# struan-robertson/shoeprint-image-retrieval

Measured on AMD Instinct MI355X. Metric: query x gallery NCC pairs/sec, higher is better.
Workload: dtype f32; 1 GPU; config 2: WVU2019-shaped VGG16 conv3_3 NCC: Q=100 x G=1500 (1500/GPU), features [256,128,64] stored as float32, rotations/scales none, queries signal 1 / noise 126; method=fft, gallery_chunk=1500, storage=float32, parallelism=gallery-shard x1, streams=1

## Files before the change

shoeprint-image-retrieval_amd/csrc/ncc_pair6.hip:

```cpp
#include <cstdlib>

#include "fft_core.h"
#include "ncc_fft_cfg.h"

namespace spr {
namespace {

#ifndef SPR_ABL
#define SPR_ABL 0
#endif
#ifndef SPR_X6
#define SPR_X6 0
#endif
#ifdef SPR_STAMPS
constexpr int kStampPoints = 12, kStampChannels = 8, kStampFirst = 8;
__device__ unsigned long long g_stamps[12 * kStampChannels * kStampPoints];
#define SPR_STAMP(i) st[i] = __builtin_amdgcn_s_memtime()
#else
#define SPR_STAMP(i)
#endif

constexpr int kTileQ6 = 16, kTileG6 = 16;

struct Pair6Args {
  int channels, nq, ng;
  int ih, iw;
  int inv_per_chan;
  int accumulate;
  int tile0;
  int tiles_g;
  int prio_mode;
  unsigned q_flags_off, g_flags_off;
};

template <int DIR>
__device__ __forceinline__ void pfa12(cf (&x)[12]) {
  constexpr float h = DIR > 0 ? 0.86602540378443860f : -0.86602540378443860f;
  cf a[3][4];
#pragma unroll
  for (int n2 = 0; n2 < 4; ++n2) {
    const cf x0 = x[(3 * n2) % 12], x1 = x[(4 + 3 * n2) % 12], x2 = x[(8 + 3 * n2) % 12];
    const cf s = x1 + x2, d = x1 - x2;
    const cf m = x0 - 0.5f * s;
    a[0][n2] = x0 + s;
    a[1][n2] = pk_iaxpy_u(d, h, m);
    a[2][n2] = pk_iaxpy_u(d, -h, m);
  }
#pragma unroll
  for (int k1 = 0; k1 < 3; ++k1) {
    const cf e0 = a[k1][0] + a[k1][2], e1 = a[k1][0] - a[k1][2];
    const cf o0 = a[k1][1] + a[k1][3], o1 = a[k1][1] - a[k1][3];
    x[(4 * k1) % 12] = e0 + o0;
    x[(4 * k1 + 18) % 12] = e0 - o0;
    x[(4 * k1 + 9) % 12] = DIR > 0 ? pk_add_i(e1, o1) : pk_sub_i(e1, o1);
    x[(4 * k1 + 27) % 12] = DIR > 0 ? pk_sub_i(e1, o1) : pk_add_i(e1, o1);
  }
}

template <class C>
struct Six {
  static_assert(C::SIX == 1 && C::EH == 12 && C::TGH == 16 && C::NW == 96 && C::NT == 384, "192 x 96 on six waves");
  static constexpr int NT = C::NT, WAVES = NT / 64;
  static constexpr int RS = 139;
  static __device__ __forceinline__ int xpos(int u) {
    if (SPR_X6 == 0) return (u / 21) * RS + u % 21;
    const int a = u < 21 ? 0 : (u < 32 ? 1 : (u < 43 ? 2 : (u < 53 ? 1 : 2)));
    const int o = u < 21 ? u : (u < 32 ? u - 11 : (u < 43 ? u - 22 : (u < 53 ? u - 43 : (u == 53 ? 9 : u - 54))));
    return a * RS + o;
  }
  static constexpr int XR = 65;
  static constexpr int XROWS = 6;
  static constexpr int kXbWave = XROWS * XR + 6;
  static constexpr int kImgOff = 0;
  static constexpr int kImgBytes = C::COLS * RS * 8;
  static constexpr int kXbOff = kImgOff + kImgBytes;
  static constexpr int kNyqOff = kXbOff + WAVES * kXbWave * 8;
  static constexpr int kHalfBytes = kNyqOff + 2 * 2 * C::NH * 8;
  static constexpr int kRedOff = 2 * kHalfBytes;
  static constexpr int kPeakOff = kRedOff + 128;
  static constexpr int kTwOff = kPeakOff + 64;
  static constexpr int kCtabOff = kTwOff + C::NH * 8;
  static constexpr int kListOff = kCtabOff + 48 * 4;
  static constexpr int kLdsBytes = kListOff;
  static_assert(kLdsBytes + 2 * 2 * 1024 <= 160 * 1024, "one workgroup of two pairs per CU, up to 1024 channels");
  static_assert(kXbOff % 8 == 0 && kNyqOff % 8 == 0 && kHalfBytes % 16 == 0 && kTwOff % 8 == 0 && kCtabOff % 8 == 0, "");
};

template <class C, bool PEAKS>
__global__ void __launch_bounds__(2 * C::NT, 3)
pair6_kernel(Pair6Args g, const unsigned char* __restrict__ pq, size_t q_item_bytes,
             const unsigned char* __restrict__ pg, size_t g_item_bytes, float* __restrict__ scores, long long ld,
             long long col0, float* __restrict__ maps_out, const cf* __restrict__ tw_h,
             const float* __restrict__ ctab, int32_t* __restrict__ peak_yx, int32_t* __restrict__ peak_tag,
             int32_t tag) {
  using S = Six<C>;
  constexpr int NT = S::NT, RS = S::RS, XR = S::XR;
  constexpr int H2 = C::EH / 2;

  constexpr int kWgPerTile = kTileQ6 * kTileG6 / 2;
  const int tile = g.tile0 + static_cast<int>(blockIdx.x) / kWgPerTile;
  const int within = static_cast<int>(blockIdx.x) % kWgPerTile;
  const int tq = tile / g.tiles_g, tg = tile - tq * g.tiles_g;
  const int half = uniform(static_cast<int>(threadIdx.x) >= NT ? 1 : 0);
  const int q_first = tq * kTileQ6 + 2 * (within >> 4);
  const int gi_item = tg * kTileG6 + 2 * (within & 7) + ((within >> 3) & 1);
  if (q_first >= g.nq || gi_item >= g.ng) return;
  const bool live = q_first + half < g.nq;
  const int qi = live ? q_first + half : q_first;

  unsigned char* lds = dyn_lds();
  unsigned char* hl = lds + half * S::kHalfBytes;
  float* red = reinterpret_cast<float*>(lds + S::kRedOff) + half * 8;
  unsigned* bar = reinterpret_cast<unsigned*>(lds + S::kRedOff + 64) + half * 8;
  unsigned* nlive_p = bar + 2;
  unsigned bar_target = 0;
  cf* R = reinterpret_cast<cf*>(hl + S::kImgOff);
  cf* nyq = reinterpret_cast<cf*>(hl + S::kNyqOff);
  cf* twt_h = reinterpret_cast<cf*>(lds + S::kTwOff);
  cf* ctab2 = reinterpret_cast<cf*>(lds + S::kCtabOff);
  unsigned short* chan = reinterpret_cast<unsigned short*>(lds + S::kListOff) + half * g.channels;

  const int tid0 = static_cast<int>(threadIdx.x) - half * NT;
  const int wv = uniform(tid0 >> 6);
  cf* xb = reinterpret_cast<cf*>(hl + S::kXbOff) + wv * S::kXbWave;

  const unsigned char* g_item = pg + static_cast<size_t>(gi_item) * g_item_bytes;
  const unsigned char* q_item = pq + static_cast<size_t>(qi) * q_item_bytes;

  if (tid0 == 0) *bar = 0u;
  if (half == 0) {
    for (int k = tid0; k < C::NH; k += NT) twt_h[k] = cconj(tw_h[(k / C::TGH) * (k % C::TGH)]);
    if (tid0 < 24) {
      const int a = (tid0 / 3) * 2, t = tid0 % 3;
      ctab2[tid0] = cmake(ctab[(3 * a + 16 * t) % 48], ctab[(3 * (a + 1) + 16 * t) % 48]);
    }
  }
  for (int k = tid0; k < g.channels; k += NT)
    chan[k] = (q_item[g.q_flags_off + k] | g_item[g.g_flags_off + k]) ? 0xFFFFu : static_cast<unsigned short>(k);
  __syncthreads();
  if (tid0 == 0) {
    int n = 0;
    for (int k = 0; k < g.channels; ++k) {
      const unsigned short v = chan[k];
      if (v != 0xFFFFu) chan[n++] = v;
    }
    if (n == 0) chan[0] = 0;
    *nlive_p = static_cast<unsigned>(n);
  }
  __syncthreads();
  const int nlive = uniform(static_cast<int>(*nlive_p));
  const int last_i = nlive > 0 ? nlive - 1 : 0;
  auto chan_at = [&](int i) { return static_cast<int>(chan[i < last_i ? i : last_i]); };

  float4 nxt[2 * H2];
  cf nyq_g, nyq_q;
  const BufRsrc g_rs = make_rsrc(g_item, g_item_bytes), q_rs = make_rsrc(q_item, q_item_bytes);
  const unsigned voff16 = static_cast<unsigned>(tid0) * 16u;
  const unsigned voff_nyq = static_cast<unsigned>(tid0 % C::NH) * 8u + C::kNyqOffset * 8u;
  constexpr unsigned kChanBytes = C::kSpecPerChan * 8u;
  const unsigned inv_base = static_cast<unsigned>(g.channels) * kChanBytes;
  auto issue_unit = [&](int c, int rc) {
    const unsigned so = static_cast<unsigned>(c) * kChanBytes + static_cast<unsigned>(rc * H2 * NT * 16);
    if (SPR_ABL == 1) {
      for (int mm = 0; mm < 2 * H2; ++mm) nxt[mm] = make_float4(0.001f * so, 0.5f, 0.25f, 0.125f);
      return;
    }
#pragma unroll
    for (int mm = 0; mm < H2; ++mm) {
      nxt[mm] = buf_ld16(g_rs, voff16, so + mm * NT * 16);
      nxt[H2 + mm] = buf_ld16(q_rs, voff16, so + mm * NT * 16);
    }
  };
  auto issue_nyq = [&](int c) {
    const unsigned so = static_cast<unsigned>(c) * kChanBytes;
    nyq_g = buf_ld8(g_rs, voff_nyq, so);
    nyq_q = buf_ld8(q_rs, voff_nyq, so);
  };
  static_assert(2 * C::NH == NT, "one Nyquist value per lane");

#ifndef SPR_EMU
  {
    const int gw = half * S::WAVES + wv;
    if (g.prio_mode == 2 && (gw == 4 || gw == 5 || gw >= 8)) __builtin_amdgcn_s_setprio(1);
  }
#endif
  cf acc[6][2];
#pragma unroll
  for (int pp = 0; pp < 6; ++pp) acc[pp][0] = acc[pp][1] = cmake(0.0f, 0.0f);

  issue_nyq(chan_at(0));
  nyq[tid0] = tid0 < C::NH ? nyq_g : nyq_q;
  issue_nyq(chan_at(1));
  nyq[NT + tid0] = tid0 < C::NH ? nyq_g : nyq_q;
  issue_unit(chan_at(0), 0);
  __syncthreads();

  for (int ci = 0; ci < nlive; ++ci) {
    const int c = chan_at(ci), c1 = chan_at(ci + 1), c2 = chan_at(ci + 2);
#ifdef SPR_STAMPS
    unsigned long long st[kStampPoints] = {};
#endif
    SPR_STAMP(0);
    const int tid = opaque(tid0);
    const int lane = tid & 63;
    const int g4 = lane >> 4, tc = lane & 15;

    auto product = [&](cf (&z)[12], int rc) {
#pragma unroll
      for (int mm = 0; mm < H2; ++mm) {
        const float4 a = nxt[mm], b = nxt[H2 + mm];
        z[2 * mm] = cmul(cmake(a.x, a.y), cmake(b.x, b.y));
        z[2 * mm + 1] = cmul(cmake(a.z, a.w), cmake(b.z, b.w));
      }
      if (rc == 0 && tid < 16) {
        const cf* nq = nyq + (ci & 1) * NT;
#pragma unroll
        for (int m = 0; m < 12; ++m) {
          const int k1 = tc + 16 * m;
          z[m] = pk_add_i(z[m], cmul(nq[k1], nq[C::NH + k1]));
        }
      }
    };
    auto stage12 = [&](cf (&z)[12]) {
      pfa12<+1>(z);
#pragma unroll
      for (int p = 1; p < 12; ++p) z[p] = cmul(z[p], twt_h[p * 16 + tc]);
    };
    auto exchange = [&](const cf (&z)[12], cf (&y)[16], int rc) {
      const int own0 = (rc * 24 + 4 * wv) * RS;
      const int xb_el = (S::kXbOff - S::kImgOff) / 8 + wv * S::kXbWave;
      const int skew = ((xb_el + 6 - own0) % 32 + 32) % 32;
      cf* own = R + own0 + skew;
      wave_sync();
      cf* w0 = xb + lane;
      cf* w1 = own + lane;
      if (SPR_ABL != 3) {
#pragma unroll
        for (int p = 0; p < 6; ++p) w0[p * XR] = z[p];
#pragma unroll
        for (int p = 6; p < 12; ++p) w1[(p - 6) * XR] = z[p];
      }
      wave_sync();
      const cf* rd = (tc < 6 ? xb + tc * XR : (tc < 12 ? own + (tc - 6) * XR : xb)) + 16 * g4;
#pragma unroll
      for (int tt = 0; tt < 16; ++tt) y[tt] = rd[tt];
    };
    auto part2 = [&](cf (&y)[16], int rc) {
      wave_sync();
      if (tc < 12) {
        if (SPR_ABL != 4) Dft<16, +1>::run(y);
        cf* col = R + (rc * 24 + 4 * wv + g4) * RS + tc;
        if (SPR_ABL != 3) {
#pragma unroll
          for (int s = 0; s < 11; ++s) col[12 * s] = y[s];
        }
      }
    };

    {
      cf za[12], ya[16], zb[12], yb[16];
      issue_nyq(c2);
      product(za, 0);
      issue_unit(c, 1);
      stage12(za);
#pragma unroll
      for (int p = 0; p < 12; ++p) pin(za[p]);
      SPR_STAMP(1);
      bar_target += S::WAVES;
      if (SPR_ABL != 2) group_barrier(bar, bar_target);
      SPR_STAMP(2);
      product(zb, 1);
      sched_fence();
      exchange(za, ya, 0);
      sched_fence();
      stage12(zb);
      sched_fence();
      issue_unit(c1, 0);
      SPR_STAMP(3);
      part2(ya, 0);
      SPR_STAMP(4);
      exchange(zb, yb, 1);
      SPR_STAMP(5);
      part2(yb, 1);
      SPR_STAMP(6);
    }
    bar_target += S::WAVES;
    if (SPR_ABL != 2) group_barrier(bar, bar_target);
    SPR_STAMP(7);
    {
      const int grp = lane / 3;
      const int t3 = lane - 3 * grp;
      const int grp_r = grp < C::kRowGroups ? grp : C::kRowGroups - 1;
      const int row = wv * C::kRowGroups + grp_r;
      const int tm = t3 == 0 ? 0 : 3 - t3;
      const cf* dbase = R + t3 * RS + row;
      const cf* mbase = R + tm * RS + row;
      const cf* cc = ctab2 + t3;
      cf z[16];
#pragma unroll
      for (int a2 = 0; a2 < 8; ++a2) {
        const cf ck = cc[a2 * 3];
#pragma unroll
        for (int h = 0; h < 2; ++h) {
          const int a = 2 * a2 + h;
          const int ra = (3 * a) % 16, rm = (3 * ((16 - a) % 16)) % 16;
          const cf av = dbase[3 * ra * RS];
          const cf bv = mbase[3 * rm * RS];
          cf v = h == 0 ? pk_conj_iaxpy<0>(av, ck, bv) : pk_conj_iaxpy<1>(av, ck, bv);
          if (a == 0) {
            const cf v0 = cmake(av.x + av.y, av.x - av.y);
            v = t3 == 0 ? v0 : v;
          }
          z[a] = v;
        }
      }
      SPR_STAMP(8);
      if (SPR_ABL != 4) Dft<16, +1>::run(z);
      sched_fence();
      float4 iv[6];
      const unsigned so_inv = inv_base + static_cast<unsigned>(c) * static_cast<unsigned>(g.inv_per_chan) * 4u;
#pragma unroll
      for (int pp = 0; pp < 6; ++pp)
        iv[pp] = SPR_ABL == 1 ? make_float4(1.f, 1.f, 1.f, 1.f) : buf_ld16(g_rs, voff16, so_inv + pp * NT * 16);
      const float kH = 0.86602540378443860f;
      const cf kl = t3 == 1 ? cmake(-0.5f, kH) : cmake(1.0f, 0.0f);
      const cf hb = t3 == 0 ? cmake(kH, 0.0f) : cmake(-kH, 0.0f);
      cf* wx = R + S::xpos(lane < 63 ? lane : 62) + wv * C::kRowGroups;
      const cf* rxt[3];
#pragma unroll
      for (int tt = 0; tt < 3; ++tt) rxt[tt] = R + S::xpos(3 * grp_r + tt) + wv * C::kRowGroups;
      wave_sync();
      if (lane < 63 && SPR_ABL != 3) {
#pragma unroll
        for (int r = 0; r < 16; ++r) wx[3 * r * RS] = z[r];
      }
      SPR_STAMP(9);
      wave_sync();
      cf yv[6][3];
#pragma unroll
      for (int pp = 0; pp < 6; ++pp)
#pragma unroll
        for (int tt = 0; tt < 3; ++tt)
          yv[pp][tt] = pp < 5 ? rxt[tt][(9 * pp + 3 * t3) * RS] : rxt[tt][45 * RS];
#pragma unroll
      for (int pp = 0; pp < 6; ++pp) {
        const cf y0 = yv[pp][0], y1 = yv[pp][1], y2 = yv[pp][2];
        const cf s = y1 + y2, d = y1 - y2;
        const cf m = y0 - 0.5f * s;
        const cf ob = pk_iaxpy<0>(d, hb, m);
        const cf oa = pk_iaxpy<1>(d, kl, pk_axpy<0>(s, kl, y0));
        const cf ia = cmake(iv[pp].x, iv[pp].y), ib = cmake(iv[pp].z, iv[pp].w);
        acc[pp][0] = oa * ia + acc[pp][0];
        acc[pp][1] = ob * ib + acc[pp][1];
        if (maps_out && half == 0) {
          const int n1 = t3 + 3 * pp;
          const int real_row = wv * C::kRowGroups + grp;
          if (n1 < 16 && grp < C::kRowGroups && real_row < g.ih) {
            const int ma = t3 == 2 ? n1 + 16 : n1, mb = t3 == 2 ? n1 : n1 + 16;
            float* dst = maps_out + (static_cast<size_t>(c) * g.ih + real_row) * g.iw;
            if (2 * ma < g.iw) dst[2 * ma] = oa.x * ia.x;
            if (2 * ma + 1 < g.iw) dst[2 * ma + 1] = oa.y * ia.y;
            if (2 * mb < g.iw) dst[2 * mb] = ob.x * ib.x;
            if (2 * mb + 1 < g.iw) dst[2 * mb + 1] = ob.y * ib.y;
          }
        }
      }
      nyq[(ci & 1) * NT + tid] = tid < C::NH ? nyq_g : nyq_q;
    }
    SPR_STAMP(10);
#ifdef SPR_STAMPS
    if (blockIdx.x == 777 && (tid0 & 63) == 0 && ci >= kStampFirst && ci < kStampFirst + kStampChannels) {
      for (int i = 0; i < kStampPoints; ++i)
        g_stamps[((half * 6 + wv) * kStampChannels + (ci - kStampFirst)) * kStampPoints + i] = st[i];
    }
#endif
  }

  if constexpr (PEAKS) {
    const int lane = tid0 & 63;
    const int grp = lane / 3, t3 = lane - 3 * grp;
    const int real_row = wv * C::kRowGroups + grp;
    const bool row_ok = grp < C::kRowGroups && real_row < g.ih;
    float best = 0.0f;
    int where = kNoPeak;
#pragma unroll
    for (int pp = 0; pp < 6; ++pp) {
      const int n1 = t3 + 3 * pp;
      const int ma = t3 == 2 ? n1 + 16 : n1, mb = t3 == 2 ? n1 : n1 + 16;
      const int at = real_row << 16;
      if (row_ok && n1 < 16) {
        if (2 * ma < g.iw) peak_take(best, where, acc[pp][0].x, at | (2 * ma));
        if (2 * ma + 1 < g.iw) peak_take(best, where, acc[pp][0].y, at | (2 * ma + 1));
        if (2 * mb < g.iw) peak_take(best, where, acc[pp][1].x, at | (2 * mb));
        if (2 * mb + 1 < g.iw) peak_take(best, where, acc[pp][1].y, at | (2 * mb + 1));
      }
    }
    wave_peak(best, where);
    int* red_pos = reinterpret_cast<int*>(lds + S::kPeakOff) + half * 8;
    if ((tid0 & 63) == 0) {
      red[wv] = best;
      red_pos[wv] = where;
    }
    __syncthreads();
    if (tid0 == 0 && live) {
      float b = red[0];
      int p = red_pos[0];
      for (int w = 1; w < S::WAVES; ++w) peak_take(b, p, red[w], red_pos[w]);
      store_peak(scores, peak_yx, peak_tag, static_cast<size_t>(qi) * ld + col0 + gi_item, b / static_cast<float>(g.channels), p,
                 tag, g.accumulate);
    }
    return;
  }
  float best = 0.0f;
#pragma unroll
  for (int pp = 0; pp < 6; ++pp) {
    best = fmaxf(best, fmaxf(fmaxf(acc[pp][0].x, acc[pp][0].y), fmaxf(acc[pp][1].x, acc[pp][1].y)));
  }
  for (int m = 32; m >= 1; m >>= 1) best = fmaxf(best, shfl_xor(best, m));
  if ((tid0 & 63) == 0) red[wv] = best;
  __syncthreads();
  if (tid0 == 0 && scores && live) {
    float b = red[0];
    for (int w = 1; w < S::WAVES; ++w) b = fmaxf(b, red[w]);
    const float s = b / static_cast<float>(g.channels);
    float* dst = scores + static_cast<size_t>(qi) * ld + col0 + gi_item;
    const float prev = g.accumulate ? *dst : 0.0f;
    *dst = s > prev ? s : prev;
  }
}

using C6 = Cfg<12, 16, 12, 8, 384, 5, 2, 1>;

}

#ifdef SPR_STAMPS
extern "C" int spr_debug_read_stamps(unsigned long long* host, int n) {
  return hipMemcpyFromSymbol(host, HIP_SYMBOL(g_stamps), sizeof(unsigned long long) * n) == hipSuccess ? 0 : -1;
}
#endif

size_t pair6_lds_bytes() { return Six<C6>::kLdsBytes; }
int pair6_max_rows() { return C6::kRows6; }
int pair6_max_cols() { return 64; }

template <bool PEAKS>
static int launch_pair6_t(const NccGeom& g, const PlanScratch& s, const PairCall& c) {
  if (!s.six_ctab) { set_error("pair6_kernel: the plan has no pre-twist table"); return SPR_ERR_ARG; }
  using S = Six<C6>;
  Pair6Args a{};
  a.channels = g.channels; a.nq = static_cast<int>(c.nq); a.ng = static_cast<int>(c.ng);
  a.ih = g.ih; a.iw = g.iw; a.inv_per_chan = g.inv_per_chan; a.accumulate = c.accumulate;
  a.tiles_g = ceil_div(static_cast<int>(c.ng), kTileG6);
  a.q_flags_off = static_cast<unsigned>(sizeof(cf) * static_cast<size_t>(g.channels) * g.spec_per_chan);
  a.g_flags_off = static_cast<unsigned>(static_cast<size_t>(g.channels) * (sizeof(cf) * g.spec_per_chan + sizeof(float) * g.inv_per_chan));
  if (g.channels > 1024) { set_error("pair6_kernel: at most 1024 channels"); return SPR_ERR_UNSUPPORTED; }
  const size_t lds_bytes = S::kLdsBytes + 2 * sizeof(unsigned short) * static_cast<size_t>(g.channels);
  a.prio_mode = env_int("SPR_P6_PRIO", 2);
  const int64_t tiles = static_cast<int64_t>(ceil_div(static_cast<int>(c.nq), kTileQ6)) * a.tiles_g;
  (void)hipFuncSetAttribute(reinterpret_cast<const void*>(pair6_kernel<C6, PEAKS>), hipFuncAttributeMaxDynamicSharedMemorySize,
                            kLdsLimit);
  const int64_t max_tiles = pair_tiles_per_launch(kTileQ6 * kTileG6 / 2, 2 * C6::NT);
  for (int64_t t0 = 0; t0 < tiles; t0 += max_tiles) {
    const int64_t n = tiles - t0 < max_tiles ? tiles - t0 : max_tiles;
    a.tile0 = static_cast<int>(t0);
    hipLaunchKernelGGL(HIP_KERNEL_NAME(pair6_kernel<C6, PEAKS>), dim3(static_cast<unsigned>(n * (kTileQ6 * kTileG6 / 2))), dim3(2 * C6::NT),
                       lds_bytes, c.stream, a, static_cast<const unsigned char*>(c.pq),
                       prepared_query_item_bytes(g, SPR_NCC_FFT), static_cast<const unsigned char*>(c.pg),
                       prepared_gallery_item_bytes(g, SPR_NCC_FFT), c.scores, static_cast<long long>(c.ld),
                       static_cast<long long>(c.col0), c.maps_out, s.tw_h, s.six_ctab, c.peak_yx, c.peak_tag, c.tag);
    const int rc = check_launch("pair6_kernel");
    if (rc != SPR_OK) return rc;
  }
  return SPR_OK;
}

int launch_pair6(const NccGeom& g, const PlanScratch& s, const PairCall& c) {
  if (c.nq == 0 || c.ng == 0) return SPR_OK;
  return c.peak_yx ? launch_pair6_t<true>(g, s, c) : launch_pair6_t<false>(g, s, c);
}

}
```

Measured before the change: 277,600 pairs/s.

## Widen LDS reads to 16 bytes for exchange rows, twiddles and pre-twist table

Re-lays out the per-wave exchange buffer (even row stride, 16-byte aligned), the twiddle table (transposed with a padded stride per lane) and the pre-twist table (grouped per t3) so that each can be read with float4 / 128-bit LDS loads instead of 8-byte loads. The Nyquist-term loads go through an opaque cursor so the compiler issues them as separate scalar LDS reads rather than merging or rescheduling them. The intent is fewer LDS instructions and less issue pressure in the FFT stages. The changed padding and skew may alter bank-conflict behaviour, and wider loads may raise register pressure.

New measurement: 279,600 pairs/s, median of 6. No clear change (+0.7%).

```diff
diff --git a/shoeprint-image-retrieval_amd/csrc/lds_solo.h b/shoeprint-image-retrieval_amd/csrc/lds_solo.h
--- /dev/null
+++ b/shoeprint-image-retrieval_amd/csrc/lds_solo.h
@@ -0,0 +1,34 @@
+#pragma once
+#include <cstddef>
+#include <cstring>
+
+#include <hip/hip_runtime.h>
+
+namespace spr {
+
+#ifdef SPR_EMU
+struct LdsCursor {
+  const unsigned char* a;
+};
+inline LdsCursor lds_cursor(const void* p) { return LdsCursor{static_cast<const unsigned char*>(p)}; }
+template <class T>
+inline T lds_ld_solo(LdsCursor& c, int byte_off) {
+  T v;
+  std::memcpy(&v, c.a + byte_off, sizeof(T));
+  return v;
+}
+#else
+struct LdsCursor {
+  unsigned a;
+};
+__device__ __forceinline__ LdsCursor lds_cursor(const void* p) {
+  return LdsCursor{static_cast<unsigned>(reinterpret_cast<size_t>((const __attribute__((address_space(3))) void*)p))};
+}
+template <class T>
+__device__ __forceinline__ T lds_ld_solo(LdsCursor& c, int byte_off) {
+  asm("" : "+v"(c.a));
+  return *reinterpret_cast<const __attribute__((address_space(3))) T*>(static_cast<size_t>(c.a + static_cast<unsigned>(byte_off)));
+}
+#endif
+
+}
diff --git a/shoeprint-image-retrieval_amd/csrc/ncc_pair6.hip b/shoeprint-image-retrieval_amd/csrc/ncc_pair6.hip
--- a/shoeprint-image-retrieval_amd/csrc/ncc_pair6.hip
+++ b/shoeprint-image-retrieval_amd/csrc/ncc_pair6.hip
@@ -1,6 +1,7 @@
 #include <cstdlib>
 
 #include "fft_core.h"
+#include "lds_solo.h"
 #include "ncc_fft_cfg.h"
 
 namespace spr {
@@ -68,9 +69,9 @@
     const int o = u < 21 ? u : (u < 32 ? u - 11 : (u < 43 ? u - 22 : (u < 53 ? u - 43 : (u == 53 ? 9 : u - 54))));
     return a * RS + o;
   }
-  static constexpr int XR = 65;
+  static constexpr int XR = 66;
   static constexpr int XROWS = 6;
-  static constexpr int kXbWave = XROWS * XR + 6;
+  static constexpr int kXbWave = XROWS * XR;
   static constexpr int kImgOff = 0;
   static constexpr int kImgBytes = C::COLS * RS * 8;
   static constexpr int kXbOff = kImgOff + kImgBytes;
@@ -79,11 +80,14 @@
   static constexpr int kRedOff = 2 * kHalfBytes;
   static constexpr int kPeakOff = kRedOff + 128;
   static constexpr int kTwOff = kPeakOff + 64;
-  static constexpr int kCtabOff = kTwOff + C::NH * 8;
+  static constexpr int TWS = 14;
+  static constexpr int kCtabOff = kTwOff + C::TGH * TWS * 8;
   static constexpr int kListOff = kCtabOff + 48 * 4;
   static constexpr int kLdsBytes = kListOff;
   static_assert(kLdsBytes + 2 * 2 * 1024 <= 160 * 1024, "one workgroup of two pairs per CU, up to 1024 channels");
-  static_assert(kXbOff % 8 == 0 && kNyqOff % 8 == 0 && kHalfBytes % 16 == 0 && kTwOff % 8 == 0 && kCtabOff % 8 == 0, "");
+  static_assert(kNyqOff % 8 == 0 && kHalfBytes % 16 == 0, "");
+  static_assert(kXbOff % 16 == 0 && kXbWave % 2 == 0 && XR % 2 == 0 && kTwOff % 16 == 0 && TWS % 2 == 0 && kCtabOff % 16 == 0,
+                "16-byte reads of the exchange rows, the twiddles and the pre-twist table");
 };
 
 template <class C, bool PEAKS>
@@ -129,10 +133,10 @@
 
   if (tid0 == 0) *bar = 0u;
   if (half == 0) {
-    for (int k = tid0; k < C::NH; k += NT) twt_h[k] = cconj(tw_h[(k / C::TGH) * (k % C::TGH)]);
+    for (int k = tid0; k < C::NH; k += NT) twt_h[(k % C::TGH) * S::TWS + k / C::TGH] = cconj(tw_h[(k / C::TGH) * (k % C::TGH)]);
     if (tid0 < 24) {
       const int a = (tid0 / 3) * 2, t = tid0 % 3;
-      ctab2[tid0] = cmake(ctab[(3 * a + 16 * t) % 48], ctab[(3 * (a + 1) + 16 * t) % 48]);
+      ctab2[t * 8 + a / 2] = cmake(ctab[(3 * a + 16 * t) % 48], ctab[(3 * (a + 1) + 16 * t) % 48]);
     }
   }
   for (int k = tid0; k < g.channels; k += NT)
@@ -213,23 +217,28 @@
         z[2 * mm + 1] = cmul(cmake(a.z, a.w), cmake(b.z, b.w));
       }
       if (rc == 0 && tid < 16) {
-        const cf* nq = nyq + (ci & 1) * NT;
+        LdsCursor nq = lds_cursor(nyq + (ci & 1) * NT + tc);
 #pragma unroll
         for (int m = 0; m < 12; ++m) {
-          const int k1 = tc + 16 * m;
-          z[m] = pk_add_i(z[m], cmul(nq[k1], nq[C::NH + k1]));
+          const cf ng = lds_ld_solo<cf>(nq, 16 * m * 8);
+          z[m] = pk_add_i(z[m], cmul(ng, lds_ld_solo<cf>(nq, (C::NH + 16 * m) * 8)));
         }
       }
     };
     auto stage12 = [&](cf (&z)[12]) {
       pfa12<+1>(z);
-#pragma unroll
-      for (int p = 1; p < 12; ++p) z[p] = cmul(z[p], twt_h[p * 16 + tc]);
+      const float4* tw4 = reinterpret_cast<const float4*>(twt_h + tc * S::TWS);
+#pragma unroll
+      for (int j = 0; j < 6; ++j) {
+        const float4 w = tw4[j];
+        if (j > 0) z[2 * j] = cmul(z[2 * j], cmake(w.x, w.y));
+        z[2 * j + 1] = cmul(z[2 * j + 1], cmake(w.z, w.w));
+      }
     };
     auto exchange = [&](const cf (&z)[12], cf (&y)[16], int rc) {
       const int own0 = (rc * 24 + 4 * wv) * RS;
       const int xb_el = (S::kXbOff - S::kImgOff) / 8 + wv * S::kXbWave;
-      const int skew = ((xb_el + 6 - own0) % 32 + 32) % 32;
+      const int skew = ((xb_el + 24 - own0) % 32 + 32) % 32;
       cf* own = R + own0 + skew;
       wave_sync();
       cf* w0 = xb + lane;
@@ -241,9 +250,13 @@
         for (int p = 6; p < 12; ++p) w1[(p - 6) * XR] = z[p];
       }
       wave_sync();
-      const cf* rd = (tc < 6 ? xb + tc * XR : (tc < 12 ? own + (tc - 6) * XR : xb)) + 16 * g4;
-#pragma unroll
-      for (int tt = 0; tt < 16; ++tt) y[tt] = rd[tt];
+      const float4* rd = reinterpret_cast<const float4*>((tc < 6 ? xb + tc * XR : (tc < 12 ? own + (tc - 6) * XR : xb)) + 16 * g4);
+#pragma unroll
+      for (int tt = 0; tt < 8; ++tt) {
+        const float4 v = rd[tt];
+        y[2 * tt] = cmake(v.x, v.y);
+        y[2 * tt + 1] = cmake(v.z, v.w);
+      }
     };
     auto part2 = [&](cf (&y)[16], int rc) {
       wave_sync();
@@ -295,11 +308,14 @@
       const int tm = t3 == 0 ? 0 : 3 - t3;
       const cf* dbase = R + t3 * RS + row;
       const cf* mbase = R + tm * RS + row;
-      const cf* cc = ctab2 + t3;
+      const f32x4* cc = reinterpret_cast<const f32x4*>(ctab2 + t3 * 8);
+      f32x4 ck4[4];
+#pragma unroll
+      for (int j = 0; j < 4; ++j) ck4[j] = cc[j];
       cf z[16];
 #pragma unroll
       for (int a2 = 0; a2 < 8; ++a2) {
-        const cf ck = cc[a2 * 3];
+        const cf ck = a2 % 2 ? __builtin_shufflevector(ck4[a2 / 2], ck4[a2 / 2], 2, 3) : __builtin_shufflevector(ck4[a2 / 2], ck4[a2 / 2], 0, 1);
 #pragma unroll
         for (int h = 0; h < 2; ++h) {
           const int a = 2 * a2 + h;
@@ -438,6 +454,16 @@
   return hipMemcpyFromSymbol(host, HIP_SYMBOL(g_stamps), sizeof(unsigned long long) * n) == hipSuccess ? 0 : -1;
 }
 #endif
+
+extern "C" int spr_debug_pair6_layout(int* out, int n) {
+  using S = Six<C6>;
+  const int v[] = {S::NT, S::WAVES, C6::COLS, C6::NH, C6::TGH, S::RS, S::XR, S::XROWS, S::kXbWave, S::kImgOff, S::kXbOff,
+                   S::kNyqOff, S::kHalfBytes, S::kRedOff, S::kPeakOff, S::kTwOff, S::kCtabOff, S::kListOff, S::kLdsBytes,
+                   C6::kRowGroups, S::TWS};
+  const int count = static_cast<int>(sizeof(v) / sizeof(v[0]));
+  for (int i = 0; i < count && i < n; ++i) out[i] = v[i];
+  return count;
+}
 
 size_t pair6_lds_bytes() { return Six<C6>::kLdsBytes; }
 int pair6_max_rows() { return C6::kRows6; }
```
